# mcarrickscott/modarith

Measured on NVIDIA B200. Metric: X25519 scalar-mults/s, higher is better.
Workload: dtype u32 limbs (saturated radix 2^32)

## Files before the change

modarith_b200/csrc/mab_capi.inc:

```
#include <cuda_runtime.h>
#include <stdlib.h>
#include <mutex>
#include <thread>
#include <vector>
#include "mab_kernels.cuh"
#include "modarith_b200.h"
#include "mab_workspace.h"
#include "mab_jit.h"
#include <string>
#include <string.h>
#include <stdio.h>

#define MAB_CAT_(a, b, c) a##b##c
#define MAB_CAT(a, b, c) MAB_CAT_(a, b, c)
#define MAB_FN(name) MAB_CAT(mab_, MAB_P, _##name)

namespace {
inline unsigned ptr_align(const void* p) {
  uintptr_t v = (uintptr_t)p;
  return (v % 16 == 0) ? 16u : (v % 8 == 0) ? 8u : (v % 4 == 0) ? 4u : 1u;
}
inline unsigned min_align(unsigned a, unsigned b) { return a < b ? a : b; }

template <int OP> int launch(const MabArgs& p, void* stream) {
// ... 451 lines not shown
  k_ecdsa_verify<MAB_F, MAB_ECDSA_ORDER><<<(unsigned)blocks, threads, smem, (cudaStream_t)stream>>>(
      (const uint8_t*)h, (const uint8_t*)r, (const uint8_t*)s, (const uint8_t*)qx, (const uint8_t*)qy, (uint8_t*)ok, n, al,
      tabws);
  er = cudaGetLastError();
  const int fr = mab_scratch_free(tabws, (cudaStream_t)stream);
  if (er == cudaSuccess && fr != 0) return fr;
  return (int)er;
}
#endif

#ifdef MAB_HAS_EDDSA
}
#include "eddsa_sm100.cuh"
#include "modarith_b200_sig.h"
extern "C" {
int mab_ED25519_eddsa_verify(const char* h, const char* sig, const char* pk, unsigned char* ok, size_t n, void* stream) {
  if (n == 0) return 0;
  typedef Eddsa<MAB_F, MAB_EDDSA_ORDER, MAB_ECN_THREADS> V;
  const int threads = MAB_ECN_THREADS;
  const size_t tab_words = (size_t)V::M::NE2W * 3 * MAB_F::L * threads;
  const size_t smem = (size_t)V::M::SCR2W * threads * sizeof(uint32_t);
  const void* kernel = (const void*)k_eddsa_verify<MAB_F, MAB_EDDSA_ORDER>;
  static int resident[64] = {0};
  int dev = 0;
  cudaError_t er = cudaGetDevice(&dev);
  if (er != cudaSuccess) return (int)er;
  if (dev < 0 || dev >= 64) return MAB_ERR_BADARG;
  if (resident[dev] == 0) {
    int sms = 0, per_sm = 0;
    if ((er = cudaFuncSetAttribute(kernel, cudaFuncAttributeMaxDynamicSharedMemorySize, (int)smem)) != cudaSuccess) return (int)er;
    if ((er = cudaDeviceGetAttribute(&sms, cudaDevAttrMultiProcessorCount, dev)) != cudaSuccess) return (int)er;
    if ((er = cudaOccupancyMaxActiveBlocksPerMultiprocessor(&per_sm, kernel, threads, smem)) != cudaSuccess) return (int)er;
    if (per_sm < 1) return MAB_ERR_BADARG;
    resident[dev] = sms * per_sm;
  }
  size_t blocks = (n + threads - 1) / threads;
  if (blocks > (size_t)resident[dev]) blocks = (size_t)resident[dev];
  const unsigned al = min_align(min_align(ptr_align(h), ptr_align(sig)), ptr_align(pk));
  uint4* tabws = nullptr;
  int rc = mab_scratch_alloc((void**)&tabws, blocks * tab_words * sizeof(uint32_t), (cudaStream_t)stream);
  if (rc != 0) return rc;
  k_eddsa_verify<MAB_F, MAB_EDDSA_ORDER><<<(unsigned)blocks, threads, smem, (cudaStream_t)stream>>>(
      (const uint8_t*)h, (const uint8_t*)sig, (const uint8_t*)pk, (uint8_t*)ok, n, al, tabws);
  er = cudaGetLastError();
  const int fr = mab_scratch_free(tabws, (cudaStream_t)stream);
  if (er == cudaSuccess && fr != 0) return fr;
  return (int)er;
}
#endif

#ifdef MAB_HAS_CURVE
}
namespace {
constexpr size_t kRoundsSmem = (size_t)(MAB_LADDER_KMAX * 3 * MAB_F::L + (MAB_F::LADDER_STASH ? 2 * MAB_F::L : 0)) *
                               MAB_LADDER_THREADS * sizeof(uint32_t);
int rounds_grid(int* grid_out, int* sms_out = nullptr) {
  static int cached[64] = {0};
  static int cached_sms[64] = {0};
  int dev = 0;
  cudaError_t e = cudaGetDevice(&dev);
  if (e != cudaSuccess) return (int)e;
  if (dev < 0 || dev >= 64) return MAB_ERR_BADARG;
  if (cached[dev] == 0) {
    int sms = 0, per_sm = 0;
    if ((e = cudaFuncSetAttribute(k_rfc7748_rounds<MAB_F>, cudaFuncAttributeMaxDynamicSharedMemorySize, (int)kRoundsSmem)) != cudaSuccess) return (int)e;
    if ((e = cudaDeviceGetAttribute(&sms, cudaDevAttrMultiProcessorCount, dev)) != cudaSuccess) return (int)e;
    if ((e = cudaOccupancyMaxActiveBlocksPerMultiprocessor(&per_sm, k_rfc7748_rounds<MAB_F>, MAB_LADDER_THREADS, kRoundsSmem)) != cudaSuccess) return (int)e;
    if (per_sm < 1) return MAB_ERR_BADARG;
    if (const char* env = getenv("MAB_LADDER_CTAS")) {
      const int v = atoi(env);
      if (v >= 1 && v < per_sm) per_sm = v;
    }
    cached_sms[dev] = sms;
    cached[dev] = sms * per_sm;
  }
  *grid_out = cached[dev];
  if (sms_out) *sms_out = cached_sms[dev];
  return 0;
}
}

extern "C" {

int MAB_FN(rfc7748)(const char* bk, const char* bu, char* bv, size_t n, void* stream) {
  if (n == 0) return 0;
  int grid = 0, sms = 0;
  int rc = rounds_grid(&grid, &sms);
  if (rc != 0) return rc;
  const int per_sm = grid / sms;
  const size_t need = (n + MAB_LADDER_THREADS - 1) / MAB_LADDER_THREADS;
  MabQueues Q;
  const size_t groups = (n + 31) / 32;
  if (groups > 0xffffffffull) return MAB_ERR_BADARG;
  Q.sms = (unsigned)sms;
  static const bool single = [] { const char* e = getenv("MAB_LADDER_QUEUES"); return e && e[0] == '1'; }();
  unsigned wq;
  if ((size_t)grid > need || single || 4 * sms > MAB_QUEUE_MAX || MAB_LADDER_THREADS != 128 || groups < (size_t)8 * sms) {
    if ((size_t)grid > need) grid = (int)need;
    Q.nq = 1;
    wq = (unsigned)grid * (MAB_LADDER_THREADS / 32);
  } else {
    Q.nq = 4u * (unsigned)sms;
    wq = (unsigned)per_sm;
  }
  Q.base = (unsigned)(groups / Q.nq);
  Q.rem = (unsigned)(groups % Q.nq);
  static const int tail = [] { const char* e = getenv("MAB_LADDER_TAIL"); return e ? atoi(e) : 1; }();
  for (int k = 0; k < 2; k++) {
    const MabQueuePlan pl = mab_queue_plan(Q.base + (unsigned)k, wq, MAB_LADDER_KMAX, tail);
    if (k == 0) { Q.c4s = pl.c4; Q.c2s = pl.c2; } else { Q.c4l = pl.c4; Q.c2l = pl.c2; }
  }
  int slot = -1;
  if ((rc = mab_queue_counters((cudaStream_t)stream, Q.nq, &Q.counter, &slot)) != 0) return rc;
  unsigned al = min_align(min_align(ptr_align(bk), ptr_align(bu)), ptr_align(bv));
  k_rfc7748_rounds<MAB_F><<<grid, MAB_LADDER_THREADS, kRoundsSmem, (cudaStream_t)stream>>>(
      (const uint8_t*)bk, (const uint8_t*)bu, (uint8_t*)bv, n, al, Q);
  cudaError_t e = cudaGetLastError();
  int r2 = mab_queue_counters_launched(slot, (cudaStream_t)stream);
  return e != cudaSuccess ? (int)e : r2;
}
int MAB_FN(rfc7748_perkey)(const char* bk, const char* bu, char* bv, size_t n, void* stream) {
  if (n == 0) return 0;
  const int threads = MAB_LADDER_THREADS;
  size_t blocks = (n + threads - 1) / threads;
  if (blocks > 0x7fffffffu) return MAB_ERR_BADARG;
  unsigned al = min_align(min_align(ptr_align(bk), ptr_align(bu)), ptr_align(bv));
  k_rfc7748<MAB_F><<<(unsigned)blocks, threads, 0, (cudaStream_t)stream>>>(
      (const uint8_t*)bk, (const uint8_t*)bu, (uint8_t*)bv, n, al);
  return (int)cudaGetLastError();
}
int MAB_FN(rfc7748_validate)(const char* bk, const char* bu, char* bv, size_t n, void* stream) {
  if (n == 0) return 0;
  const int threads = MAB_LADDER_THREADS;
  size_t blocks = (n + threads - 1) / threads;
  if (blocks > 0x7fffffffu) return MAB_ERR_BADARG;
  unsigned al = min_align(min_align(ptr_align(bk), ptr_align(bu)), ptr_align(bv));
  k_rfc7748<MAB_F, true><<<(unsigned)blocks, threads, 0, (cudaStream_t)stream>>>(
      (const uint8_t*)bk, (const uint8_t*)bu, (uint8_t*)bv, n, al);
  return (int)cudaGetLastError();
}

static const void* mab_device_view(const void* p) {
  cudaPointerAttributes a;
  if (cudaPointerGetAttributes(&a, p) != cudaSuccess) { cudaGetLastError(); return nullptr; }
  return (a.type == cudaMemoryTypeHost) ? a.devicePointer : nullptr;
}
int MAB_FN(rfc7748_host)(const char* bk, const char* bu, char* bv, size_t n, int device) {
  if (n == 0) return 0;
  cudaError_t e;
  int prev = 0;
  if ((e = cudaGetDevice(&prev)) != cudaSuccess) return (int)e;
  if ((e = cudaSetDevice(device)) != cudaSuccess) return (int)e;
  const size_t NB = MAB_F::NBYTES;
  const int NS = MAB_WS_STREAMS;
  {
    const char* zc = getenv("MAB_HOST_ZEROCOPY");
    const void *dk = nullptr, *du = nullptr, *dv = nullptr;
    if (!(zc && zc[0] == '0') && (dk = mab_device_view(bk)) && (du = mab_device_view(bu)) && (dv = mab_device_view(bv)) &&
        mab_device_view(bk + n * NB - 1) && mab_device_view(bu + n * NB - 1) && mab_device_view(bv + n * NB - 1)) {
      MabWorkspace* ws = nullptr;
      int rc = mab_host_workspace_acquire(device, 0, &ws);
      if (rc == 0) {
        rc = MAB_FN(rfc7748)((const char*)dk, (const char*)du, (char*)dv, n, ws->stream[0]);
        e = cudaStreamSynchronize(ws->stream[0]);
        if (rc == 0 && e != cudaSuccess) rc = (int)e;
        mab_host_workspace_release(ws);
      }
      cudaSetDevice(prev);
      return rc;
    }
  }
  int grid = 0;
// ... 61 lines not shown
```

modarith_b200/csrc/mab_kernels.cuh:

```cuda
#pragma once
#include "mab_queue_plan.h"
#include <cuda_runtime.h>
#include "modarith_b200.h"
#include "rfc7748_sm100.cuh"
#include "weierstrass_sm100.cuh"
#include "edwards_sm100.cuh"

enum MabOp {
  OP_ADD, OP_SUB, OP_NEG, OP_MUL, OP_SQR, OP_MLI, OP_CPY, OP_NSQR, OP_PRO, OP_INV, OP_INVH,
  OP_QR, OP_QRH, OP_SQRT, OP_SQRTH, OP_IS1, OP_IS0, OP_ZER, OP_ONE, OP_INT, OP_NRES, OP_REDC,
  OP_CSW, OP_CMV, OP_SHL, OP_SHR, OP_HAF, OP_2R, OP_SIGN, OP_CMP, OP_FSB, OP_MULCHAIN
};

struct MabArgs {
  const uint32_t* a;
  const uint32_t* b;
  uint32_t* r;
  uint32_t* r2;
  int* iout;
  const int* iin;
  uint32_t scalar;
  size_t n, stride;
};

// ... 251 lines not shown
    }
  }
}

template <class F> __global__ void __launch_bounds__(128) k_imp(const uint8_t* bytes, uint32_t* r, int* status, size_t n, size_t stride, unsigned align) {
  constexpr int L = F::L;
  size_t i = (size_t)blockIdx.x * blockDim.x + threadIdx.x;
  if (i >= n) return;
  uint32_t w[L], a[L];
  if constexpr (F::NBYTES == 4 * L) {
    uint32_t raw[L];
    aos_ld<L>(raw, bytes, i, align);
#pragma unroll
    for (int j = 0; j < L; j++) w[j] = mab_bswap(raw[L - 1 - j]);
  } else {
    const uint8_t* e = bytes + i * (size_t)F::NBYTES;
#pragma unroll
    for (int j = 0; j < L; j++) w[j] = 0;
#pragma unroll
    for (int b = 0; b < F::NBYTES; b++) {
      const int pos = F::NBYTES - 1 - b;
      w[pos >> 2] |= (uint32_t)e[b] << (8 * (pos & 3));
    }
  }
  uint32_t lt = Field<F>::from_words(a, w);
  plane_st<L>(r, stride, i, a);
  if (status) status[i] = (int)lt;
}
template <class F> __global__ void __launch_bounds__(128) k_exp(const uint32_t* ap, uint8_t* bytes, size_t n, size_t stride, unsigned align) {
  constexpr int L = F::L;
  size_t i = (size_t)blockIdx.x * blockDim.x + threadIdx.x;
  if (i >= n) return;
  uint32_t a[L], w[L];
  plane_ld<L>(a, ap, stride, i);
  Field<F>::to_words(w, a);
  if constexpr (F::NBYTES == 4 * L) {
    uint32_t raw[L];
#pragma unroll
    for (int j = 0; j < L; j++) raw[L - 1 - j] = mab_bswap(w[j]);
    aos_st<L>(bytes, i, align, raw);
  } else {
    uint8_t* e = bytes + i * (size_t)F::NBYTES;
#pragma unroll
    for (int b = 0; b < F::NBYTES; b++) {
      const int pos = F::NBYTES - 1 - b;
      e[b] = (uint8_t)(w[pos >> 2] >> (8 * (pos & 3)));
    }
  }
}

#ifndef MAB_LADDER_THREADS
#define MAB_LADDER_THREADS 128
#endif
#ifdef MAB_LADDER_MINBLOCKS
#define MAB_LADDER_BOUNDS(F) __launch_bounds__(MAB_LADDER_THREADS, MAB_LADDER_MINBLOCKS)
#else
#define MAB_LADDER_BOUNDS(F) __launch_bounds__(MAB_LADDER_THREADS, F::LADDER_MINBLOCKS)
#endif
template <class F, bool VALIDATE = false> __global__ void MAB_LADDER_BOUNDS(F) k_rfc7748(const uint8_t* bk, const uint8_t* bu, uint8_t* bv, size_t n, unsigned align) {
  constexpr int L = F::L;
  static_assert(F::NBYTES == 4 * L, "byte strings are whole words for the supported curves");
  size_t i = (size_t)blockIdx.x * blockDim.x + threadIdx.x;
  if (i >= n) return;
  uint32_t k[L], u[L], out[L];
  aos_ld<L>(k, bk, i, align);
  aos_ld<L>(u, bu, i, align);
  if constexpr (F::LADDER_STASH) {
    __shared__ uint32_t stash[2 * L][MAB_LADDER_THREADS];
    Rfc7748<F>::template scalarmult<VALIDATE>(out, k, u, &stash[0][threadIdx.x], MAB_LADDER_THREADS);
  } else {
    Rfc7748<F>::template scalarmult<VALIDATE>(out, k, u);
  }
  aos_st<L>(bv, i, align, out);
}

#ifndef MAB_LADDER_KMAX
#define MAB_LADDER_KMAX 4
#endif
struct MabQueues {
  unsigned long long* counter;
  unsigned nq;
  unsigned sms;
  unsigned base, rem;
  unsigned c4s, c2s, c4l, c2l;
};
static __device__ __forceinline__ void mab_queue_range(const MabQueues& Q, unsigned q, unsigned long long& lo, unsigned& g, unsigned& longer) {
  longer = q < Q.rem ? 1u : 0u;
  lo = (unsigned long long)q * Q.base + (q < Q.rem ? q : Q.rem);
  g = Q.base + longer;
}
template <class F> __global__ void MAB_LADDER_BOUNDS(F) k_rfc7748_rounds(const uint8_t* bk, const uint8_t* bu, uint8_t* bv, size_t n, unsigned align, MabQueues Q) {
  constexpr int L = F::L;
  constexpr int T = MAB_LADDER_THREADS;
  extern __shared__ uint32_t mab_smem[];
  uint32_t* st = mab_smem + threadIdx.x;
  uint32_t* stash = F::LADDER_STASH ? (mab_smem + MAB_LADDER_KMAX * 3 * L * T + threadIdx.x) : nullptr;
  const unsigned lane = threadIdx.x & 31;
  constexpr unsigned AT_HOME = 0xffffffffu;
  unsigned swept = AT_HOME;
  for (;;) {
    unsigned home = 0;
    if (Q.nq > 1) {
      unsigned smid;
      asm("mov.u32 %0, %%smid;" : "=r"(smid));
      while (smid >= Q.sms) smid -= Q.sms;
      home = smid * 4 + ((threadIdx.x >> 5) & 3);
    }
    int K = 0;
    unsigned first = 0;
    unsigned long long glo = 0;
    for (;;) {
      unsigned q = home;
      if (swept != AT_HOME) {
        bool found = false;
        while (swept + 1 < Q.nq) {
          const unsigned cand = swept + 1 + lane;
          int has = 0;
          if (cand < Q.nq) {
            unsigned qq = home + cand;
            if (qq >= Q.nq) qq -= Q.nq;
            unsigned long long lo2; unsigned g2, lg2;
            mab_queue_range(Q, qq, lo2, g2, lg2);
            const unsigned c4 = lg2 ? Q.c4l : Q.c4s, c2 = lg2 ? Q.c2l : Q.c2s;
            has = *(volatile unsigned long long*)(Q.counter + qq) < (unsigned long long)mab_queue_nchunks(g2, c4, c2);
          }
          const unsigned m = __ballot_sync(0xffffffffu, has);
          if (m) {
            swept += (unsigned)(__ffs((int)m) - 1);
            q = home + swept + 1;
            if (q >= Q.nq) q -= Q.nq;
            found = true;
            break;
          }
          swept += 32;
        }
        if (!found) break;
      }
      unsigned g, longer;
      mab_queue_range(Q, q, glo, g, longer);
      const unsigned c4 = longer ? Q.c4l : Q.c4s, c2 = longer ? Q.c2l : Q.c2s;
      const unsigned nchunks = mab_queue_nchunks(g, c4, c2);
      unsigned long long ci = 0;
      int ok = 0;
      if (lane == 0) {
        if (*(volatile unsigned long long*)(Q.counter + q) < (unsigned long long)nchunks) {
          ci = atomicAdd(Q.counter + q, 1ULL);
          ok = 1;
        }
      }
      ok = __shfl_sync(0xffffffffu, ok, 0);
      if (ok) {
        ci = __shfl_sync(0xffffffffu, ci, 0);
        K = mab_queue_chunk(g, c4, c2, ci, first);
        if (K) break;
      }
      swept = (swept == AT_HOME) ? 0 : swept + 1;
      if (Q.nq == 1) break;
    }
    if (!K) break;
    const size_t start = (size_t)(glo + first) * 32;
    MAB_NOUNROLL
    for (int j = 0; j < K; j++) {
      const size_t idx = start + (size_t)j * 32 + lane;
      uint32_t k[L], u[L], x1[L], x2[L], z2[L];
      if (idx < n) {
        aos_ld<L>(k, bk, idx, align);
        aos_ld<L>(u, bu, idx, align);
      } else {
#pragma unroll
        for (int w = 0; w < L; w++) { k[w] = 0; u[w] = 0; }
      }
      Rfc7748<F>::ladder(x2, z2, x1, k, u, stash, T);
      Rfc7748<F>::st_(st, T, j, 0, x2);
      Rfc7748<F>::st_(st, T, j, 1, z2);
    }
    Rfc7748<F>::finish_batch(st, T, K);
    MAB_NOUNROLL
    for (int j = 0; j < K; j++) {
      const size_t idx = start + (size_t)j * 32 + lane;
      if (idx < n) {
        uint32_t out[L];
        Rfc7748<F>::ld(out, st, T, j, 0);
        aos_st<L>(bv, idx, align, out);
      }
    }
  }
}

#ifdef MAB_ECN_GLOBAL_TABLE
#define MAB_ECN_GLOBAL(G) (MAB_ECN_GLOBAL_TABLE != 0)
#else
#define MAB_ECN_GLOBAL(G) (G::ECN_GLOBAL_TABLE)
#endif
#ifdef MAB_ECN_MINBLOCKS
#define MAB_ECN_MB(G) (MAB_ECN_MINBLOCKS)
#else
#define MAB_ECN_MB(G) (G::ECN_MINBLOCKS)
#endif
#ifdef MAB_ECN2_MINBLOCKS
#define MAB_ECN2_MB(G) (MAB_ECN2_MINBLOCKS)
#else
#define MAB_ECN2_MB(G) (G::ECN2_MINBLOCKS)
#endif
#define MAB_ECN_THREADS 128
template <class F, class G> __global__ void __launch_bounds__(MAB_ECN_THREADS, MAB_ECN_MB(G))
k_ecnmul(const uint8_t* e, const uint8_t* x, const uint8_t* y, uint8_t* xo, uint8_t* yo, size_t n, unsigned align,
         uint4* tabws) {
  constexpr int L = F::L;
  static_assert(F::NBYTES == 4 * L, "whole-word byte strings");
  extern __shared__ uint4 mab_smem4[];
  typedef EcnMul<G, MAB_ECN_THREADS> M;
  uint4* tab;
  uint32_t* scr;
  if (MAB_ECN_GLOBAL(G)) {
    tab = tabws + (size_t)blockIdx.x * (9 * 3 * (L / 4) * MAB_ECN_THREADS) + threadIdx.x;
    scr = reinterpret_cast<uint32_t*>(mab_smem4) + threadIdx.x;
  } else {
    tab = mab_smem4 + threadIdx.x;
    scr = nullptr;
  }
  for (size_t blk = blockIdx.x; blk * MAB_ECN_THREADS < n; blk += gridDim.x) {
    const size_t i = blk * MAB_ECN_THREADS + threadIdx.x;
    if (i >= n) break;
    uint32_t raw[L], ew[L], xw[L], yw[L];
    aos_ld<L>(raw, e, i, align);
#pragma unroll
    for (int j = 0; j < L; j++) ew[j] = mab_bswap(raw[L - 1 - j]);
    aos_ld<L>(raw, x, i, align);
#pragma unroll
    for (int j = 0; j < L; j++) xw[j] = mab_bswap(raw[L - 1 - j]);
    aos_ld<L>(raw, y, i, align);
#pragma unroll
    for (int j = 0; j < L; j++) yw[j] = mab_bswap(raw[L - 1 - j]);
    typename G::Pt P;
    G::set(P, xw, yw);
    M::mul(P, ew, tab, MAB_ECN_THREADS, scr, align >> 16);
    G::get(xw, yw, P);
// ... 65 lines not shown
```

modarith_b200/csrc/mab_queue_plan.h:

```cpp
#pragma once
#if defined(__CUDACC__)
#define MAB_HD __host__ __device__ __forceinline__
#else
#define MAB_HD inline
#endif

struct MabQueuePlan {
  unsigned c4, c2;
};

MAB_HD MabQueuePlan mab_queue_plan(unsigned g, unsigned w, int kmax, int tail) {
  MabQueuePlan p;
  p.c4 = (kmax >= 4 && g > w) ? (g - w) / (4 * w) * w : 0;
  const unsigned left = g - 4 * p.c4;
  p.c2 = (left > w) ? (left - w) / (2 * w) * w : 0;
  if (tail == 2 || (tail == 1 && p.c4 == 0)) p.c2 = left / (2 * w) * w;
  return p;
}

MAB_HD unsigned mab_queue_nchunks(unsigned g, unsigned c4, unsigned c2) { return c4 + c2 + (g - 4 * c4 - 2 * c2); }

MAB_HD int mab_queue_chunk(unsigned g, unsigned c4, unsigned c2, unsigned long long ci, unsigned& first) {
  if (ci < c4) { first = (unsigned)ci * 4; return 4; }
  if (ci < (unsigned long long)c4 + c2) { first = c4 * 4 + (unsigned)(ci - c4) * 2; return 2; }
  const unsigned long long s = (unsigned long long)c4 * 4 + (unsigned long long)c2 * 2 + (ci - c4 - c2);
  if (s >= g) return 0;
  first = (unsigned)s;
  return 1;
}
```

modarith_b200/csrc/mab_runtime.cu:

```cuda
#include <cuda_runtime.h>
#include <string.h>
#include <stdio.h>
#include "modarith_b200.h"
#include "gen/field_X25519.cuh"
#include "gen/field_X448.cuh"
#include "gen/field_NIST256.cuh"
#include "mab_probe.cuh"
#include "mab_workspace.h"
#include "mab_jit.h"
#include "mab_unsat29.cuh"
#include <mutex>

#define NCH 8
template <int VARIANT> __global__ void __launch_bounds__(256) k_imad_peak(const uint32_t* seed, uint32_t* sink, int iters) {
  uint32_t x = seed[threadIdx.x & 31], y = seed[32 + (threadIdx.x & 31)];
  uint32_t lo[NCH], hi[NCH], al[NCH];
#pragma unroll
  for (int c = 0; c < NCH; c++) { lo[c] = x + c; hi[c] = y ^ c; al[c] = x * c; }
  for (int it = 0; it < iters; it++) {
#pragma unroll
    for (int u = 0; u < 4; u++) {
      if (VARIANT == 0) {
#pragma unroll
        for (int c = 0; c < NCH; c++)
// ... 35 lines not shown
        for (int c = 0; c < NCH; c++) {
          asm volatile("add.u32 %0, %0, %1;" : "+r"(lo[c]) : "r"(x));
          asm volatile("add.u32 %0, %0, %1;" : "+r"(hi[c]) : "r"(y));
        }
      }
    }
  }
  uint32_t acc = 0;
#pragma unroll
  for (int c = 0; c < NCH; c++) acc ^= lo[c] ^ hi[c] ^ al[c];
  if (acc == 0x12345678u) sink[0] = acc;
}

template <int V> static void launch_probe(int v, int blocks, int threads, cudaStream_t st, const uint32_t* d, uint32_t* sink, int iters) {
  if (v == V) k_probe<V><<<blocks, threads, 0, st>>>(d, sink, iters);
  if constexpr (V + 1 < MAB_NPROBE) launch_probe<V + 1>(v, blocks, threads, st, d, sink, iters);
}

static MabWorkspace g_ws[MAB_WS_MAXDEV];
static std::mutex g_ws_mutex[MAB_WS_MAXDEV];

int mab_host_workspace_acquire(int device, size_t bytes, MabWorkspace** out) {
  if (device < 0 || device >= MAB_WS_MAXDEV) return MAB_ERR_BADARG;
  g_ws_mutex[device].lock();
  MabWorkspace* ws = &g_ws[device];
  cudaError_t e = cudaSuccess;
  if (!ws->ready) {
    for (int s = 0; s < MAB_WS_STREAMS && e == cudaSuccess; s++) {
      ws->buf[s] = nullptr;
      e = cudaStreamCreateWithFlags(&ws->stream[s], cudaStreamNonBlocking);
    }
    ws->bytes = 0;
    ws->device = device;
    ws->ready = (e == cudaSuccess);
  }
  if (e == cudaSuccess && ws->bytes < bytes) {
    for (int s = 0; s < MAB_WS_STREAMS && e == cudaSuccess; s++) {
      if (ws->buf[s]) cudaFree(ws->buf[s]);
      ws->buf[s] = nullptr;
      e = cudaMalloc((void**)&ws->buf[s], bytes);
    }
    ws->bytes = (e == cudaSuccess) ? bytes : 0;
  }
  if (e != cudaSuccess) {
    g_ws_mutex[device].unlock();
    return (int)e;
  }
  *out = ws;
  return 0;
}

void mab_host_workspace_release(MabWorkspace* ws) { g_ws_mutex[ws->device].unlock(); }

#define MAB_NSLOTS 256
struct MabCounterSlot {
  cudaEvent_t done;
  bool used;
};
static unsigned long long* g_counters[MAB_WS_MAXDEV];
static MabCounterSlot* g_slots[MAB_WS_MAXDEV];
static unsigned g_counter_next[MAB_WS_MAXDEV];
static std::mutex g_counter_mutex;

int mab_queue_counters(cudaStream_t stream, unsigned nq, unsigned long long** out, int* slot) {
  if (nq == 0 || nq > MAB_QUEUE_MAX) return MAB_ERR_BADARG;
  int dev = 0;
  cudaError_t e = cudaGetDevice(&dev);
  if (e != cudaSuccess) return (int)e;
  if (dev < 0 || dev >= MAB_WS_MAXDEV) return MAB_ERR_BADARG;
  unsigned id;
  {
    std::lock_guard<std::mutex> g(g_counter_mutex);
    if (!g_counters[dev]) {
      if ((e = cudaMalloc((void**)&g_counters[dev], (size_t)MAB_NSLOTS * MAB_QUEUE_MAX * sizeof(unsigned long long))) != cudaSuccess) return (int)e;
      g_slots[dev] = new MabCounterSlot[MAB_NSLOTS];
      for (int i = 0; i < MAB_NSLOTS; i++) {
        g_slots[dev][i].used = false;
        if ((e = cudaEventCreateWithFlags(&g_slots[dev][i].done, cudaEventDisableTiming)) != cudaSuccess) return (int)e;
      }
    }
    id = g_counter_next[dev]++ % MAB_NSLOTS;
    if (g_slots[dev][id].used && (e = cudaStreamWaitEvent(stream, g_slots[dev][id].done, 0)) != cudaSuccess) return (int)e;
    g_slots[dev][id].used = true;
  }
  unsigned long long* p = g_counters[dev] + (size_t)id * MAB_QUEUE_MAX;
  if ((e = cudaMemsetAsync(p, 0, (size_t)nq * sizeof(unsigned long long), stream)) != cudaSuccess) return (int)e;
  *out = p;
  *slot = (int)id;
  return 0;
}

int mab_queue_counters_launched(int slot, cudaStream_t stream) {
  int dev = 0;
  cudaError_t e = cudaGetDevice(&dev);
  if (e != cudaSuccess) return (int)e;
  if (dev < 0 || dev >= MAB_WS_MAXDEV || slot < 0 || slot >= MAB_NSLOTS || !g_slots[dev]) return MAB_ERR_BADARG;
  std::lock_guard<std::mutex> g(g_counter_mutex);
  return (int)cudaEventRecord(g_slots[dev][slot].done, stream);
}

static cudaMemPool_t g_pool[MAB_WS_MAXDEV];
static bool g_pool_ready[MAB_WS_MAXDEV];
static std::mutex g_pool_mutex;

int mab_scratch_alloc(void** out, size_t bytes, cudaStream_t stream) {
  int dev = 0;
  cudaError_t e = cudaGetDevice(&dev);
  if (e != cudaSuccess) return (int)e;
  if (dev < 0 || dev >= MAB_WS_MAXDEV) return MAB_ERR_BADARG;
  {
    std::lock_guard<std::mutex> g(g_pool_mutex);
    if (!g_pool_ready[dev]) {
      cudaMemPoolProps props = {};
      props.allocType = cudaMemAllocationTypePinned;
      props.handleTypes = cudaMemHandleTypeNone;
      props.location.type = cudaMemLocationTypeDevice;
      props.location.id = dev;
      if ((e = cudaMemPoolCreate(&g_pool[dev], &props)) != cudaSuccess) return (int)e;
      unsigned long long keep = ~0ull;
      if ((e = cudaMemPoolSetAttribute(g_pool[dev], cudaMemPoolAttrReleaseThreshold, &keep)) != cudaSuccess) return (int)e;
      g_pool_ready[dev] = true;
    }
  }
  return (int)cudaMallocFromPoolAsync(out, bytes, g_pool[dev], stream);
}

int mab_scratch_free(void* p, cudaStream_t stream) { return (int)cudaFreeAsync(p, stream); }

static const char* kVersion = "modarith_b200 0.1 (sm_100a)";

template <class F> static long long products_of(const char* what) {
  const long long L = F::L, M = L * L, S = L * (L + 1) / 2, I = L;
  const long long pro = F::PRO_SQR * S + F::PRO_MUL * M;
  const long long inv_wrap = (F::PM1D2 - 1) * (S + M) + (F::PM1D2 + 1) * S + M;
  if (!strcmp(what, "modmul")) return M;
  if (!strcmp(what, "modsqr")) return S;
  if (!strcmp(what, "modmli")) return I;
  if (!strcmp(what, "modpro")) return pro;
  if (!strcmp(what, "modinv")) return pro + inv_wrap;
  if (!strcmp(what, "modsqrt")) {
    long long w = pro + M;
    if (F::PM1D2 > 1) {
      w += M;
      for (int k = F::PM1D2; k > 1; k--) w += (k - 2) * S + 2 * M + S;
    }
    return w;
  }
  if (!strcmp(what, "rfc7748") && F::HAS_CURVE)
    return (long long)F::NBITS * (5 * M + 4 * S + I) + pro + inv_wrap + M + (F::MONTGOMERY ? 4 * M : 0);
  return -1;
}

extern "C" {

const char* mab_version(void) { return kVersion; }

const char* mab_error_string(int code) {
  if (code == 0) return "ok";
  if (code == MAB_ERR_BADARG) return "modarith_b200: bad argument";
  if (code == MAB_ERR_NODEVICE) return "modarith_b200: no CUDA device";
  if (code == MAB_ERR_NOJIT) return "modarith_b200: NVRTC (libnvrtc.so.12) could not be loaded; see mab_jit_log()";
  if (code == MAB_ERR_JIT) return "modarith_b200: run-time compilation failed; see mab_jit_log()";
  return cudaGetErrorString((cudaError_t)code);
}

void mab_release_workspaces(void) {
  mab_jit_release();
  {
    std::lock_guard<std::mutex> g(g_counter_mutex);
    int prev = 0;
    cudaGetDevice(&prev);
    for (int d = 0; d < MAB_WS_MAXDEV; d++) {
      if (!g_counters[d]) continue;
      cudaSetDevice(d);
      cudaDeviceSynchronize();
      for (int i = 0; i < MAB_NSLOTS; i++) cudaEventDestroy(g_slots[d][i].done);
      delete[] g_slots[d];
      g_slots[d] = nullptr;
      cudaFree(g_counters[d]);
      g_counters[d] = nullptr;
      g_counter_next[d] = 0;
    }
    cudaSetDevice(prev);
  }
  {
    std::lock_guard<std::mutex> g(g_pool_mutex);
    for (int d = 0; d < MAB_WS_MAXDEV; d++)
      if (g_pool_ready[d]) {
        cudaMemPoolDestroy(g_pool[d]);
        g_pool_ready[d] = false;
      }
  }
  for (int d = 0; d < MAB_WS_MAXDEV; d++) {
    std::lock_guard<std::mutex> g(g_ws_mutex[d]);
    MabWorkspace* ws = &g_ws[d];
    if (!ws->ready) continue;
    int prev = 0;
    cudaGetDevice(&prev);
    cudaSetDevice(d);
    for (int s = 0; s < MAB_WS_STREAMS; s++) {
      if (ws->buf[s]) cudaFree(ws->buf[s]);
      cudaStreamDestroy(ws->stream[s]);
      ws->buf[s] = nullptr;
    }
    ws->bytes = 0;
    ws->ready = false;
    cudaSetDevice(prev);
  }
}

int mab_device_count(void) {
  int n = 0;
  if (cudaGetDeviceCount(&n) != cudaSuccess) { cudaGetLastError(); return 0; }
  return n;
}

int mab_params(const char* prime, int* wordlength, int* nlimbs, int* radix, int* nbits, int* nbytes) {
  int L, nb, by;
  if (!strcmp(prime, "X25519")) { L = F_X25519::L; nb = F_X25519::NBITS; by = F_X25519::NBYTES; }
  else if (!strcmp(prime, "X448")) { L = F_X448::L; nb = F_X448::NBITS; by = F_X448::NBYTES; }
  else if (!strcmp(prime, "NIST256")) { L = F_NIST256::L; nb = F_NIST256::NBITS; by = F_NIST256::NBYTES; }
  else return MAB_ERR_BADARG;
  if (wordlength) *wordlength = 32;
  if (nlimbs) *nlimbs = L;
  if (radix) *radix = 32;
  if (nbits) *nbits = nb;
  if (nbytes) *nbytes = by;
  return 0;
}

long long mab_products(const char* prime, const char* what) {
  if (!strcmp(prime, "X25519")) return products_of<F_X25519>(what);
  if (!strcmp(prime, "X448")) return products_of<F_X448>(what);
  if (!strcmp(prime, "NIST256")) return products_of<F_NIST256>(what);
  return -1;
}

int mab_imad_peak(int variant, int iters, int blocks, int threads, float* ms, double* instructions, void* stream) {
  if (iters <= 0 || blocks <= 0 || threads <= 0 || threads > 256) return MAB_ERR_BADARG;
  cudaStream_t st = (cudaStream_t)stream;
  uint32_t host[64];
  for (int i = 0; i < 64; i++) host[i] = 0x9e3779b9u * (i + 1) | 1u;
  uint32_t* d = nullptr;
  cudaError_t e = cudaMalloc((void**)&d, 65 * sizeof(uint32_t));
// ... 72 lines not shown
```

modarith_b200/csrc/mab_workspace.h:

```cpp
#pragma once
#include <cuda_runtime.h>
#include <stddef.h>
#define MAB_WS_STREAMS 3
#define MAB_WS_MAXDEV 64
struct MabWorkspace {
  cudaStream_t stream[MAB_WS_STREAMS];
  char* buf[MAB_WS_STREAMS];
  size_t bytes;
  int device;
  bool ready;
};
int mab_host_workspace_acquire(int device, size_t bytes, MabWorkspace** out);
void mab_host_workspace_release(MabWorkspace* ws);
#define MAB_QUEUE_MAX 1024
int mab_queue_counters(cudaStream_t stream, unsigned nq, unsigned long long** out, int* slot);
int mab_queue_counters_launched(int slot, cudaStream_t stream);
int mab_scratch_alloc(void** out, size_t bytes, cudaStream_t stream);
int mab_scratch_free(void* p, cudaStream_t stream);
```

modarith_b200/csrc/rfc7748_sm100.cuh:

```cuda
#pragma once
#include "mab_field.cuh"

#ifdef MAB_STEP_UNROLL2
#define MAB_STEP_UNROLL _Pragma("unroll 2")
#else
#define MAB_STEP_UNROLL MAB_NOUNROLL
#endif
#ifdef MAB_NO_TAIL_DOUBLING
#define MAB_TAIL_DOUBLINGS(F) 0
#else
#define MAB_TAIL_DOUBLINGS(F) (F::COF)
#endif

template <class F> struct Rfc7748 {
  static constexpr int L = F::L;
  typedef Field<F> Fd;

  static MAB_DEV void clamp(uint32_t (&k)[L]) {
    constexpr int s = (8 - (F::NBITS % 8)) % 8;
    k[0] &= ~((1u << F::COF) - 1u);
    constexpr uint32_t topmask = ((0xffu >> s) << 24) | 0x00ffffffu;
    k[L - 1] &= topmask;
    k[L - 1] |= (0x80u >> s) << 24;
  }
// ... 80 lines not shown
    for (int i = 0; i < MAB_TAIL_DOUBLINGS(F); i++) {
      uint32_t A[L], B[L];
      F::add_tt(A, x2, z2);
      F::sub_tt(B, x2, z2);
      F::sqr(A, A);
      F::sqr(B, B);
      F::mul(x2, A, B);
      F::sub_tt(B, A, B);
      F::mla(z2, B, F::A24, A);
      F::mul(z2, z2, B);
    }
  }

  template <bool VALIDATE>
  static MAB_DEV void tail(uint32_t (&out)[L], uint32_t (&x2)[L], uint32_t (&z2)[L], const uint32_t (&x1)[L],
                           uint32_t* stash, int pitch) {
    if (!VALIDATE) {
      uint32_t h[L];
      F::pro(h, z2);
      Fd::template inv<true>(z2, z2, h);
    } else {
      uint32_t A[L], B[L], C[L], D[L], E[L], w[L];
      if (stash) {
#pragma unroll
        for (int j = 0; j < L; j++) w[j] = stash[(L + j) * pitch];
      } else {
        Fd::cpy(w, x1);
      }
      F::mul(B, w, z2);
      F::mul(A, B, z2);
      F::pro(E, A);
      Fd::cpy(C, A);
      F::mul(D, E, z2);
      F::sqr(D, D);
      F::mul(D, D, w);
#pragma unroll
      for (int i = 0; i < F::COF - 2; i++) { F::sqr(C, C); F::mul(C, C, A); }
#pragma unroll
      for (int i = 0; i < F::COF; i++) F::sqr(E, E);
      F::mul(C, C, E);
      F::mul(z2, C, B);
#pragma unroll
      for (int i = 0; i < F::COF - 2; i++) F::sqr(D, D);
      Fd::one(A);
      F::add(D, D, A);
      (void)Fd::fsb(D);
      (void)Fd::shr(D, 1);
      F::mul(x2, x2, D);
    }
    F::mul(x2, x2, z2);
    Fd::to_words(out, x2);
  }

  static MAB_DEV void finish_batch(uint32_t* st, int pitch, int K) {
    uint32_t acc[L], z[L], t[L], one[L];
    Fd::one(one);
    uint32_t flags = 0;
    MAB_NOUNROLL
    for (int j = 0; j < K; j++) {
      ld(z, st, pitch, j, 1);
      uint32_t f = Fd::is0_stored(z);
      flags |= f << j;
      Fd::cmv(f, one, z);
      st_(st, pitch, j, 1, z);
      if (j == 0) Fd::cpy(acc, z); else F::mul(acc, acc, z);
      st_(st, pitch, j, 2, acc);
    }
    {
      uint32_t h[L];
      F::pro(h, acc);
      Fd::template inv<true>(acc, acc, h);
    }
    MAB_NOUNROLL
    for (int j = K - 1; j >= 0; j--) {
      if (j > 0) {
        ld(t, st, pitch, j - 1, 2);
        F::mul(t, acc, t);
        ld(z, st, pitch, j, 1);
        F::mul(acc, acc, z);
      } else {
        Fd::cpy(t, acc);
      }
      ld(z, st, pitch, j, 0);
      F::mul(z, z, t);
      uint32_t zero[L];
      Fd::zer(zero);
      Fd::cmv((flags >> j) & 1u, zero, z);
      Fd::to_words(t, z);
      st_(st, pitch, j, 0, t);
    }
  }
  static MAB_DEV void ld(uint32_t (&r)[L], const uint32_t* st, int pitch, int j, int e) {
#pragma unroll
    for (int w = 0; w < L; w++) r[w] = st[((j * 3 + e) * L + w) * pitch];
  }
  static MAB_DEV void st_(uint32_t* st, int pitch, int j, int e, const uint32_t (&r)[L]) {
#pragma unroll
    for (int w = 0; w < L; w++) st[((j * 3 + e) * L + w) * pitch] = r[w];
  }
};
```

Measured before the change: 53.03 million.

## Decouple ladder work items from batched inversion via global scratch and item counters

Each warp now claims a single 32-key group per atomic instead of variable chunks of up to four, and stores the ladder's projective (x,z) results to global scratch instead of shared memory. A per-item arrival counter lets the last warp to finish a KI-group item (default 16) run the Montgomery batch inversion over that whole item. Batching 16 groups per inversion spreads the single field inversion over more keys, and dropping the shared-memory staging can raise occupancy. In exchange it adds global-memory round trips, threadfences and a memset per launch, plus chunked launches for very large n. The finish_batch rewrite also stores partial products in the x slot so only two stored elements per key are needed instead of three.

Result: no change. 53.16 million, median of 6 (+0.3%).

```diff
diff --git a/modarith_b200/csrc/mab_capi.inc b/modarith_b200/csrc/mab_capi.inc
--- a/modarith_b200/csrc/mab_capi.inc
+++ b/modarith_b200/csrc/mab_capi.inc
@@ -527,8 +527,7 @@
 #ifdef MAB_HAS_CURVE
 }
 namespace {
-constexpr size_t kRoundsSmem = (size_t)(MAB_LADDER_KMAX * 3 * MAB_F::L + (MAB_F::LADDER_STASH ? 2 * MAB_F::L : 0)) *
-                               MAB_LADDER_THREADS * sizeof(uint32_t);
+constexpr size_t kRoundsSmem = (size_t)(MAB_F::LADDER_STASH ? 2 * MAB_F::L : 0) * MAB_LADDER_THREADS * sizeof(uint32_t);
 int rounds_grid(int* grid_out, int* sms_out = nullptr) {
   static int cached[64] = {0};
   static int cached_sms[64] = {0};
@@ -557,42 +556,49 @@
 
 extern "C" {
 
+static int rounds_launch(const char* bk, const char* bu, char* bv, size_t n, cudaStream_t stream, int grid, int sms,
+                         unsigned* ws, size_t cnt_words) {
+  const size_t need = (n + MAB_LADDER_THREADS - 1) / MAB_LADDER_THREADS;
+  const size_t groups = (n + 31) / 32;
+  MabQueues Q;
+  Q.sms = (unsigned)sms;
+  static const bool single = [] { const char* e = getenv("MAB_LADDER_QUEUES"); return e && e[0] == '1'; }();
+  unsigned nq = 4u * (unsigned)sms;
+  if ((size_t)grid > need || single || MAB_LADDER_THREADS != 128 || groups < (size_t)8 * sms) {
+    if ((size_t)grid > need) grid = (int)need;
+    nq = 1;
+  }
+  Q.P = mab_plan(groups, nq, MAB_LADDER_KI);
+  const size_t ncnt = nq + (size_t)mab_item_base(Q.P, nq);
+  if (ncnt > cnt_words) return MAB_ERR_BADARG;
+  Q.counter = ws;
+  Q.scr = ws + cnt_words;
+  cudaError_t e = cudaMemsetAsync(Q.counter, 0, ncnt * sizeof(unsigned), stream);
+  if (e != cudaSuccess) return (int)e;
+  unsigned al = min_align(min_align(ptr_align(bk), ptr_align(bu)), ptr_align(bv));
+  k_rfc7748_rounds<MAB_F><<<grid, MAB_LADDER_THREADS, kRoundsSmem, stream>>>(
+      (const uint8_t*)bk, (const uint8_t*)bu, (uint8_t*)bv, n, al, Q);
+  return (int)cudaGetLastError();
+}
+
 int MAB_FN(rfc7748)(const char* bk, const char* bu, char* bv, size_t n, void* stream) {
   if (n == 0) return 0;
   int grid = 0, sms = 0;
   int rc = rounds_grid(&grid, &sms);
   if (rc != 0) return rc;
-  const int per_sm = grid / sms;
-  const size_t need = (n + MAB_LADDER_THREADS - 1) / MAB_LADDER_THREADS;
-  MabQueues Q;
-  const size_t groups = (n + 31) / 32;
-  if (groups > 0xffffffffull) return MAB_ERR_BADARG;
-  Q.sms = (unsigned)sms;
-  static const bool single = [] { const char* e = getenv("MAB_LADDER_QUEUES"); return e && e[0] == '1'; }();
-  unsigned wq;
-  if ((size_t)grid > need || single || 4 * sms > MAB_QUEUE_MAX || MAB_LADDER_THREADS != 128 || groups < (size_t)8 * sms) {
-    if ((size_t)grid > need) grid = (int)need;
-    Q.nq = 1;
-    wq = (unsigned)grid * (MAB_LADDER_THREADS / 32);
-  } else {
-    Q.nq = 4u * (unsigned)sms;
-    wq = (unsigned)per_sm;
-  }
-  Q.base = (unsigned)(groups / Q.nq);
-  Q.rem = (unsigned)(groups % Q.nq);
-  static const int tail = [] { const char* e = getenv("MAB_LADDER_TAIL"); return e ? atoi(e) : 1; }();
-  for (int k = 0; k < 2; k++) {
-    const MabQueuePlan pl = mab_queue_plan(Q.base + (unsigned)k, wq, MAB_LADDER_KMAX, tail);
-    if (k == 0) { Q.c4s = pl.c4; Q.c2s = pl.c2; } else { Q.c4l = pl.c4; Q.c2l = pl.c2; }
-  }
-  int slot = -1;
-  if ((rc = mab_queue_counters((cudaStream_t)stream, Q.nq, &Q.counter, &slot)) != 0) return rc;
-  unsigned al = min_align(min_align(ptr_align(bk), ptr_align(bu)), ptr_align(bv));
-  k_rfc7748_rounds<MAB_F><<<grid, MAB_LADDER_THREADS, kRoundsSmem, (cudaStream_t)stream>>>(
-      (const uint8_t*)bk, (const uint8_t*)bu, (uint8_t*)bv, n, al, Q);
-  cudaError_t e = cudaGetLastError();
-  int r2 = mab_queue_counters_launched(slot, (cudaStream_t)stream);
-  return e != cudaSuccess ? (int)e : r2;
+  const size_t m = n < (size_t)MAB_LADDER_LAUNCH_KEYS ? n : (size_t)MAB_LADDER_LAUNCH_KEYS;
+  const size_t groups = (m + 31) / 32;
+  const size_t cnt_words = (4 * (size_t)sms + groups + 31) / 32 * 32;
+  const size_t bytes = (cnt_words + groups * 32 * 2 * MAB_F::L) * sizeof(uint32_t);
+  unsigned* ws = nullptr;
+  if ((rc = mab_scratch_alloc((void**)&ws, bytes, (cudaStream_t)stream)) != 0) return rc;
+  const size_t NB = MAB_F::NBYTES;
+  for (size_t off = 0; off < n && rc == 0; off += m) {
+    const size_t c = (n - off < m) ? n - off : m;
+    rc = rounds_launch(bk + off * NB, bu + off * NB, bv + off * NB, c, (cudaStream_t)stream, grid, sms, ws, cnt_words);
+  }
+  const int fr = mab_scratch_free(ws, (cudaStream_t)stream);
+  return rc != 0 ? rc : fr;
 }
 int MAB_FN(rfc7748_perkey)(const char* bk, const char* bu, char* bv, size_t n, void* stream) {
   if (n == 0) return 0;
diff --git a/modarith_b200/csrc/mab_kernels.cuh b/modarith_b200/csrc/mab_kernels.cuh
--- a/modarith_b200/csrc/mab_kernels.cuh
+++ b/modarith_b200/csrc/mab_kernels.cuh
@@ -327,6 +327,11 @@
 #ifndef MAB_LADDER_THREADS
 #define MAB_LADDER_THREADS 128
 #endif
+#ifndef MAB_LADDER_KI
+#define MAB_LADDER_KI 16
+#endif
+static_assert(MAB_LADDER_KI >= 1 && MAB_LADDER_KI <= 32, "one zero flag per key of an inversion item in 32 bits");
+#define MAB_LADDER_LAUNCH_KEYS (1u << 24)
 #ifdef MAB_LADDER_MINBLOCKS
 #define MAB_LADDER_BOUNDS(F) __launch_bounds__(MAB_LADDER_THREADS, MAB_LADDER_MINBLOCKS)
 #else
@@ -349,61 +354,51 @@
   aos_st<L>(bv, i, align, out);
 }
 
-#ifndef MAB_LADDER_KMAX
-#define MAB_LADDER_KMAX 4
-#endif
 struct MabQueues {
-  unsigned long long* counter;
-  unsigned nq;
+  unsigned* counter;
+  uint32_t* scr;
   unsigned sms;
-  unsigned base, rem;
-  unsigned c4s, c2s, c4l, c2l;
+  MabPlan P;
 };
-static __device__ __forceinline__ void mab_queue_range(const MabQueues& Q, unsigned q, unsigned long long& lo, unsigned& g, unsigned& longer) {
-  longer = q < Q.rem ? 1u : 0u;
-  lo = (unsigned long long)q * Q.base + (q < Q.rem ? q : Q.rem);
-  g = Q.base + longer;
-}
 template <class F> __global__ void MAB_LADDER_BOUNDS(F) k_rfc7748_rounds(const uint8_t* bk, const uint8_t* bu, uint8_t* bv, size_t n, unsigned align, MabQueues Q) {
   constexpr int L = F::L;
   constexpr int T = MAB_LADDER_THREADS;
   extern __shared__ uint32_t mab_smem[];
-  uint32_t* st = mab_smem + threadIdx.x;
-  uint32_t* stash = F::LADDER_STASH ? (mab_smem + MAB_LADDER_KMAX * 3 * L * T + threadIdx.x) : nullptr;
+  uint32_t* stash = F::LADDER_STASH ? (mab_smem + threadIdx.x) : nullptr;
   const unsigned lane = threadIdx.x & 31;
+  unsigned* items = Q.counter + Q.P.nq;
   constexpr unsigned AT_HOME = 0xffffffffu;
   unsigned swept = AT_HOME;
   for (;;) {
     unsigned home = 0;
-    if (Q.nq > 1) {
+    if (Q.P.nq > 1) {
       unsigned smid;
       asm("mov.u32 %0, %%smid;" : "=r"(smid));
       while (smid >= Q.sms) smid -= Q.sms;
       home = smid * 4 + ((threadIdx.x >> 5) & 3);
     }
-    int K = 0;
-    unsigned first = 0;
+    bool got = false;
+    unsigned q = home, g = 0, j = 0;
     unsigned long long glo = 0;
     for (;;) {
-      unsigned q = home;
+      q = home;
       if (swept != AT_HOME) {
         bool found = false;
-        while (swept + 1 < Q.nq) {
+        while (swept + 1 < Q.P.nq) {
           const unsigned cand = swept + 1 + lane;
           int has = 0;
-          if (cand < Q.nq) {
+          if (cand < Q.P.nq) {
             unsigned qq = home + cand;
-            if (qq >= Q.nq) qq -= Q.nq;
-            unsigned long long lo2; unsigned g2, lg2;
-            mab_queue_range(Q, qq, lo2, g2, lg2);
-            const unsigned c4 = lg2 ? Q.c4l : Q.c4s, c2 = lg2 ? Q.c2l : Q.c2s;
-            has = *(volatile unsigned long long*)(Q.counter + qq) < (unsigned long long)mab_queue_nchunks(g2, c4, c2);
+            if (qq >= Q.P.nq) qq -= Q.P.nq;
+            unsigned long long lo2; unsigned g2;
+            mab_queue_range(Q.P, qq, lo2, g2);
+            has = *(volatile unsigned*)(Q.counter + qq) < g2;
           }
           const unsigned m = __ballot_sync(0xffffffffu, has);
           if (m) {
             swept += (unsigned)(__ffs((int)m) - 1);
             q = home + swept + 1;
-            if (q >= Q.nq) q -= Q.nq;
+            if (q >= Q.P.nq) q -= Q.P.nq;
             found = true;
             break;
           }
@@ -411,32 +406,26 @@
         }
         if (!found) break;
       }
-      unsigned g, longer;
-      mab_queue_range(Q, q, glo, g, longer);
-      const unsigned c4 = longer ? Q.c4l : Q.c4s, c2 = longer ? Q.c2l : Q.c2s;
-      const unsigned nchunks = mab_queue_nchunks(g, c4, c2);
-      unsigned long long ci = 0;
+      mab_queue_range(Q.P, q, glo, g);
       int ok = 0;
       if (lane == 0) {
-        if (*(volatile unsigned long long*)(Q.counter + q) < (unsigned long long)nchunks) {
-          ci = atomicAdd(Q.counter + q, 1ULL);
-          ok = 1;
+        if (*(volatile unsigned*)(Q.counter + q) < g) {
+          j = atomicAdd(Q.counter + q, 1u);
+          ok = j < g;
         }
       }
       ok = __shfl_sync(0xffffffffu, ok, 0);
       if (ok) {
-        ci = __shfl_sync(0xffffffffu, ci, 0);
-        K = mab_queue_chunk(g, c4, c2, ci, first);
-        if (K) break;
+        j = __shfl_sync(0xffffffffu, j, 0);
+        got = true;
+        break;
       }
       swept = (swept == AT_HOME) ? 0 : swept + 1;
-      if (Q.nq == 1) break;
-    }
-    if (!K) break;
-    const size_t start = (size_t)(glo + first) * 32;
-    MAB_NOUNROLL
-    for (int j = 0; j < K; j++) {
-      const size_t idx = start + (size_t)j * 32 + lane;
+      if (Q.P.nq == 1) break;
+    }
+    if (!got) break;
+    {
+      const size_t idx = (size_t)(glo + j) * 32 + lane;
       uint32_t k[L], u[L], x1[L], x2[L], z2[L];
       if (idx < n) {
         aos_ld<L>(k, bk, idx, align);
@@ -446,18 +435,28 @@
         for (int w = 0; w < L; w++) { k[w] = 0; u[w] = 0; }
       }
       Rfc7748<F>::ladder(x2, z2, x1, k, u, stash, T);
-      Rfc7748<F>::st_(st, T, j, 0, x2);
-      Rfc7748<F>::st_(st, T, j, 1, z2);
-    }
-    Rfc7748<F>::finish_batch(st, T, K);
-    MAB_NOUNROLL
-    for (int j = 0; j < K; j++) {
-      const size_t idx = start + (size_t)j * 32 + lane;
-      if (idx < n) {
-        uint32_t out[L];
-        Rfc7748<F>::ld(out, st, T, j, 0);
-        aos_st<L>(bv, idx, align, out);
-      }
+      uint32_t* col = Q.scr + (size_t)(glo + j) * (2 * L * 32) + lane;
+      Rfc7748<F>::st_(col, 32, 0, 0, x2);
+      Rfc7748<F>::st_(col, 32, 0, 1, z2);
+    }
+    __threadfence();
+    __syncwarp();
+    unsigned first = 0, size = 0;
+    int ready = 0;
+    if (lane == 0) {
+      const unsigned long long it = mab_item_of(Q.P, q, j, first, size);
+      ready = atomicAdd(items + it, 1u) == size - 1;
+    }
+    if (__shfl_sync(0xffffffffu, ready, 0)) {
+      __threadfence();
+      first = __shfl_sync(0xffffffffu, first, 0);
+      size = __shfl_sync(0xffffffffu, size, 0);
+      const unsigned long long g0 = glo + first;
+      Rfc7748<F>::finish_batch(Q.scr + (size_t)g0 * (2 * L * 32) + lane, 32, (int)size,
+                               [&](int jj, const uint32_t (&w)[L]) {
+                                 const size_t idx = (size_t)(g0 + (unsigned)jj) * 32 + lane;
+                                 if (idx < n) aos_st<L>(bv, idx, align, w);
+                               });
     }
   }
 }
diff --git a/modarith_b200/csrc/mab_queue_plan.h b/modarith_b200/csrc/mab_queue_plan.h
--- a/modarith_b200/csrc/mab_queue_plan.h
+++ b/modarith_b200/csrc/mab_queue_plan.h
@@ -4,6 +4,39 @@
 #else
 #define MAB_HD inline
 #endif
+
+struct MabPlan {
+  unsigned nq;
+  unsigned base, rem;
+  unsigned ki;
+};
+
+MAB_HD MabPlan mab_plan(unsigned long long groups, unsigned nq, unsigned ki) {
+  MabPlan p;
+  p.nq = nq;
+  p.base = (unsigned)(groups / nq);
+  p.rem = (unsigned)(groups % nq);
+  p.ki = ki;
+  return p;
+}
+
+MAB_HD void mab_queue_range(const MabPlan& P, unsigned q, unsigned long long& lo, unsigned& g) {
+  lo = (unsigned long long)q * P.base + (q < P.rem ? q : P.rem);
+  g = P.base + (q < P.rem ? 1u : 0u);
+}
+
+MAB_HD unsigned long long mab_item_base(const MabPlan& P, unsigned q) {
+  const unsigned long long nl = (P.base + 1 + P.ki - 1) / P.ki, ns = (P.base + P.ki - 1) / P.ki;
+  return q < P.rem ? (unsigned long long)q * nl : (unsigned long long)P.rem * nl + (unsigned long long)(q - P.rem) * ns;
+}
+
+MAB_HD unsigned long long mab_item_of(const MabPlan& P, unsigned q, unsigned j, unsigned& first, unsigned& size) {
+  const unsigned g = P.base + (q < P.rem ? 1u : 0u);
+  const unsigned it = j / P.ki;
+  first = it * P.ki;
+  size = (g - first < P.ki) ? g - first : P.ki;
+  return mab_item_base(P, q) + it;
+}
 
 struct MabQueuePlan {
   unsigned c4, c2;
diff --git a/modarith_b200/csrc/mab_runtime.cu b/modarith_b200/csrc/mab_runtime.cu
--- a/modarith_b200/csrc/mab_runtime.cu
+++ b/modarith_b200/csrc/mab_runtime.cu
@@ -111,53 +111,6 @@
 
 void mab_host_workspace_release(MabWorkspace* ws) { g_ws_mutex[ws->device].unlock(); }
 
-#define MAB_NSLOTS 256
-struct MabCounterSlot {
-  cudaEvent_t done;
-  bool used;
-};
-static unsigned long long* g_counters[MAB_WS_MAXDEV];
-static MabCounterSlot* g_slots[MAB_WS_MAXDEV];
-static unsigned g_counter_next[MAB_WS_MAXDEV];
-static std::mutex g_counter_mutex;
-
-int mab_queue_counters(cudaStream_t stream, unsigned nq, unsigned long long** out, int* slot) {
-  if (nq == 0 || nq > MAB_QUEUE_MAX) return MAB_ERR_BADARG;
-  int dev = 0;
-  cudaError_t e = cudaGetDevice(&dev);
-  if (e != cudaSuccess) return (int)e;
-  if (dev < 0 || dev >= MAB_WS_MAXDEV) return MAB_ERR_BADARG;
-  unsigned id;
-  {
-    std::lock_guard<std::mutex> g(g_counter_mutex);
-    if (!g_counters[dev]) {
-      if ((e = cudaMalloc((void**)&g_counters[dev], (size_t)MAB_NSLOTS * MAB_QUEUE_MAX * sizeof(unsigned long long))) != cudaSuccess) return (int)e;
-      g_slots[dev] = new MabCounterSlot[MAB_NSLOTS];
-      for (int i = 0; i < MAB_NSLOTS; i++) {
-        g_slots[dev][i].used = false;
-        if ((e = cudaEventCreateWithFlags(&g_slots[dev][i].done, cudaEventDisableTiming)) != cudaSuccess) return (int)e;
-      }
-    }
-    id = g_counter_next[dev]++ % MAB_NSLOTS;
-    if (g_slots[dev][id].used && (e = cudaStreamWaitEvent(stream, g_slots[dev][id].done, 0)) != cudaSuccess) return (int)e;
-    g_slots[dev][id].used = true;
-  }
-  unsigned long long* p = g_counters[dev] + (size_t)id * MAB_QUEUE_MAX;
-  if ((e = cudaMemsetAsync(p, 0, (size_t)nq * sizeof(unsigned long long), stream)) != cudaSuccess) return (int)e;
-  *out = p;
-  *slot = (int)id;
-  return 0;
-}
-
-int mab_queue_counters_launched(int slot, cudaStream_t stream) {
-  int dev = 0;
-  cudaError_t e = cudaGetDevice(&dev);
-  if (e != cudaSuccess) return (int)e;
-  if (dev < 0 || dev >= MAB_WS_MAXDEV || slot < 0 || slot >= MAB_NSLOTS || !g_slots[dev]) return MAB_ERR_BADARG;
-  std::lock_guard<std::mutex> g(g_counter_mutex);
-  return (int)cudaEventRecord(g_slots[dev][slot].done, stream);
-}
-
 static cudaMemPool_t g_pool[MAB_WS_MAXDEV];
 static bool g_pool_ready[MAB_WS_MAXDEV];
 static std::mutex g_pool_mutex;
@@ -226,29 +179,17 @@
 void mab_release_workspaces(void) {
   mab_jit_release();
   {
-    std::lock_guard<std::mutex> g(g_counter_mutex);
+    std::lock_guard<std::mutex> g(g_pool_mutex);
     int prev = 0;
     cudaGetDevice(&prev);
-    for (int d = 0; d < MAB_WS_MAXDEV; d++) {
-      if (!g_counters[d]) continue;
-      cudaSetDevice(d);
-      cudaDeviceSynchronize();
-      for (int i = 0; i < MAB_NSLOTS; i++) cudaEventDestroy(g_slots[d][i].done);
-      delete[] g_slots[d];
-      g_slots[d] = nullptr;
-      cudaFree(g_counters[d]);
-      g_counters[d] = nullptr;
-      g_counter_next[d] = 0;
-    }
-    cudaSetDevice(prev);
-  }
-  {
-    std::lock_guard<std::mutex> g(g_pool_mutex);
     for (int d = 0; d < MAB_WS_MAXDEV; d++)
       if (g_pool_ready[d]) {
+        cudaSetDevice(d);
+        cudaDeviceSynchronize();
         cudaMemPoolDestroy(g_pool[d]);
         g_pool_ready[d] = false;
       }
+    cudaSetDevice(prev);
   }
   for (int d = 0; d < MAB_WS_MAXDEV; d++) {
     std::lock_guard<std::mutex> g(g_ws_mutex[d]);
diff --git a/modarith_b200/csrc/mab_workspace.h b/modarith_b200/csrc/mab_workspace.h
--- a/modarith_b200/csrc/mab_workspace.h
+++ b/modarith_b200/csrc/mab_workspace.h
@@ -12,8 +12,5 @@
 };
 int mab_host_workspace_acquire(int device, size_t bytes, MabWorkspace** out);
 void mab_host_workspace_release(MabWorkspace* ws);
-#define MAB_QUEUE_MAX 1024
-int mab_queue_counters(cudaStream_t stream, unsigned nq, unsigned long long** out, int* slot);
-int mab_queue_counters_launched(int slot, cudaStream_t stream);
 int mab_scratch_alloc(void** out, size_t bytes, cudaStream_t stream);
 int mab_scratch_free(void* p, cudaStream_t stream);
diff --git a/modarith_b200/csrc/rfc7748_sm100.cuh b/modarith_b200/csrc/rfc7748_sm100.cuh
--- a/modarith_b200/csrc/rfc7748_sm100.cuh
+++ b/modarith_b200/csrc/rfc7748_sm100.cuh
@@ -156,19 +156,24 @@
     Fd::to_words(out, x2);
   }
 
-  static MAB_DEV void finish_batch(uint32_t* st, int pitch, int K) {
-    uint32_t acc[L], z[L], t[L], one[L];
+  template <class Out> static MAB_DEV void finish_batch(uint32_t* st, int pitch, int K, Out out) {
+    uint32_t acc[L], x[L], z[L], one[L];
     Fd::one(one);
     uint32_t flags = 0;
     MAB_NOUNROLL
     for (int j = 0; j < K; j++) {
       ld(z, st, pitch, j, 1);
-      uint32_t f = Fd::is0_stored(z);
+      const uint32_t f = Fd::is0_stored(z);
       flags |= f << j;
       Fd::cmv(f, one, z);
-      st_(st, pitch, j, 1, z);
-      if (j == 0) Fd::cpy(acc, z); else F::mul(acc, acc, z);
-      st_(st, pitch, j, 2, acc);
+      if (j == 0) {
+        Fd::cpy(acc, z);
+      } else {
+        ld(x, st, pitch, j, 0);
+        F::mul(x, x, acc);
+        st_(st, pitch, j, 0, x);
+        F::mul(acc, acc, z);
+      }
     }
     {
       uint32_t h[L];
@@ -177,29 +182,35 @@
     }
     MAB_NOUNROLL
     for (int j = K - 1; j >= 0; j--) {
+      ld(x, st, pitch, j, 0);
+      F::mul(x, x, acc);
       if (j > 0) {
-        ld(t, st, pitch, j - 1, 2);
-        F::mul(t, acc, t);
         ld(z, st, pitch, j, 1);
+        Fd::cmv((flags >> j) & 1u, one, z);
         F::mul(acc, acc, z);
-      } else {
-        Fd::cpy(t, acc);
-      }
-      ld(z, st, pitch, j, 0);
-      F::mul(z, z, t);
-      uint32_t zero[L];
-      Fd::zer(zero);
-      Fd::cmv((flags >> j) & 1u, zero, z);
-      Fd::to_words(t, z);
-      st_(st, pitch, j, 0, t);
-    }
+      }
+      Fd::zer(z);
+      Fd::cmv((flags >> j) & 1u, z, x);
+      uint32_t w[L];
+      Fd::to_words(w, x);
+      out(j, w);
+    }
+  }
+  static MAB_DEV void finish_batch(uint32_t* st, int pitch, int K) {
+    finish_batch(st, pitch, K, [&](int j, const uint32_t (&w)[L]) { st_(st, pitch, j, 0, w); });
   }
   static MAB_DEV void ld(uint32_t (&r)[L], const uint32_t* st, int pitch, int j, int e) {
 #pragma unroll
-    for (int w = 0; w < L; w++) r[w] = st[((j * 3 + e) * L + w) * pitch];
+    for (int w = 0; w < L; w++) {
+#ifdef MAB_HOSTSIM
+      r[w] = st[((j * 2 + e) * L + w) * pitch];
+#else
+      r[w] = __ldcg(st + ((j * 2 + e) * L + w) * pitch);
+#endif
+    }
   }
   static MAB_DEV void st_(uint32_t* st, int pitch, int j, int e, const uint32_t (&r)[L]) {
 #pragma unroll
-    for (int w = 0; w < L; w++) st[((j * 3 + e) * L + w) * pitch] = r[w];
+    for (int w = 0; w < L; w++) st[((j * 2 + e) * L + w) * pitch] = r[w];
   }
 };
```
